# astra-vision/rain-rendering

Measured on AMD Instinct MI355X. Metric: rainy frames/sec @ 1242x375, 100 mm/hr, higher is better.
Workload: dtype f64 alpha/mask, f32 colour

## Files before the change

rain-rendering_amd/csrc/rainhip.hip:

```cpp
#include <hip/hip_runtime.h>

#include <dlfcn.h>

#include <cstddef>
#include <cstdio>
#include <cstdlib>
#include <algorithm>
#include <cstring>
#include <string>
#include <type_traits>
#include <mutex>
#include <unordered_map>
#include <vector>

#include "rainhip.h"
#include "rr_device.h"
#include "rr_prepass.h"
#include "rr_deflate.h"
#include "rr_pngrows.h"
#include "rr_particles.h"
#include "rr_lens.h"
#include "rr_resize.h"
#include "rr_convert.h"

// ... 696 lines not shown
  }
#pragma unroll
  for (int c = 0; c < NCH; c++) {
    const int y = c * 64 + lane;
    if (y < Hp) {
      uint32_t* out = sc.spans + ((int64_t)f * Hp + y) * Dp;
#pragma unroll
      for (int k = 0; k < FOV_GROUPS; k++)
        if (have[k]) out[dk[k]] = packed[k][c];
    }
  }
  if (!from_list) break;
  wave_lds_sync();
  }
}

#ifndef RR_DDA_WAVES
#define RR_DDA_WAVES 1
#endif
constexpr int DDA_WAVES = RR_DDA_WAVES;
template <int CTRL, int ROW_MASK>
__device__ inline int dpp_keep_i32(int v) { return __builtin_amdgcn_update_dpp(v, v, CTRL, ROW_MASK, 0xf, false); }
__device__ inline int wave_min_scan_i32(int v) {
  v = imin(v, dpp_keep_i32<0x111, 0xf>(v));
  v = imin(v, dpp_keep_i32<0x112, 0xf>(v));
  v = imin(v, dpp_keep_i32<0x114, 0xf>(v));
  v = imin(v, dpp_keep_i32<0x118, 0xf>(v));
  v = imin(v, dpp_keep_i32<0x142, 0xa>(v));
  v = imin(v, dpp_keep_i32<0x143, 0xc>(v));
  return v;
}
__device__ inline int wave_max_scan_i32(int v) {
  v = imax(v, dpp_keep_i32<0x111, 0xf>(v));
  v = imax(v, dpp_keep_i32<0x112, 0xf>(v));
  v = imax(v, dpp_keep_i32<0x114, 0xf>(v));
  v = imax(v, dpp_keep_i32<0x118, 0xf>(v));
  v = imax(v, dpp_keep_i32<0x142, 0xa>(v));
  v = imax(v, dpp_keep_i32<0x143, 0xc>(v));
  return v;
}

constexpr uint32_t FOV_KEY_LAST = 0xffffu;
__global__ __launch_bounds__(64 * DDA_WAVES) void k_fov_vertices(const FrameDesc* frames, Dims dm, rr_camera cam, int max_drops, int ordered, Scratch sc) {
  const int f = blockIdx.y, wave = threadIdx.x >> 6, lane = threadIdx.x & 63;
  const FrameDesc& fr = frames[f];
  const int N = cam.n_fov;
  const int i = (blockIdx.x * DDA_WAVES + wave) * 64 + lane;
  const bool act = i < fr.n_drops;
  const int64_t gi = (int64_t)f * max_drops + (act ? i : 0);
  if (fr.strategy == 1) {
    if (act) {
      sc.npts[gi] = -1;
      sc.fov_rec[gi] = make_uint4(0u, 0u, 0u, (ordered ? FOV_KEY_LAST : 0u) << 16);
    }
    return;
  }
  uint32_t* const gpix = sc.fov_pix + (int64_t)f * N * max_drops + (act ? i : 0);
  auto pixv = [&](int kk) -> uint32_t& { return gpix[(int64_t)kk * max_drops]; };
  uint32_t top_xy = 0;
  int uns = 0;
  int count_true = 0, count_false = 0;
  int ktop = 0, ytop = 1 << 30, ybot = -(1 << 30), r_first = 0;
  bool spread = false, on_map = true;
  int turns = 0, dir = 0, dir_first = 0;
  float dist = 0.f;
  if (act) {
    FovSetup32 F;
    const rr_drop d = load_drop(fr.drops + i);
    fov_setup32(d, (float)cam.fov_cos, (float)cam.fov_sin, F, uns);
    dist = sqrtf(F.pos[0] * F.pos[0] + F.pos[1] * F.pos[1] + F.pos[2] * F.pos[2]);
    float az_prev = 0.f, er_prev = 0.f, az0 = 0.f, er0 = 0.f;
    int y_prev = 0, y0v = 0;
    for (int k = 0; k < N; k++) {
      float az, er, pxf, pyf;
      fov_vertex32(F, (float)cam.radius, (float)cam.phi_cos[k], (float)cam.phi_sin[k], dm.He, dm.We, az, er, pxf, pyf, uns);
      const int ix = (int)pxf, iy = (int)pyf;
      const uint32_t vxy = (uint32_t)(ix & 0xffff) | ((uint32_t)(iy & 0xffff) << 16);
      pixv(k) = vxy;
      on_map = on_map && ix >= 0 && ix < dm.We && iy >= 0 && iy < dm.He;
      const int r = imin(imax(iy, 0), dm.He - 1);
      if (k == 0) { az0 = az; er0 = er; r_first = r; y0v = iy; }
      else {
        const bool c = fov_wrap_cnd32(az_prev, az, er_prev, er, uns);
        count_true += c ? 1 : 0;
        count_false += c ? 0 : 1;
        spread = spread || iabs(r - r_first) >= 2;
        const int sg = iy > y_prev ? 1 : (iy < y_prev ? -1 : 0);
        if (sg != 0) {
          if (dir == 0) dir_first = sg;
          else if (sg != dir) turns++;
          dir = sg;
        }
      }
      if (iy < ytop) { ytop = iy; ktop = k; top_xy = vxy; }
      ybot = imax(ybot, iy);
      az_prev = az; er_prev = er; y_prev = iy;
    }
    {
      const bool c = fov_wrap_cnd32(az_prev, az0, er_prev, er0, uns);
      count_true += c ? 1 : 0;
      count_false += c ? 0 : 1;
      const int sg = y0v > y_prev ? 1 : (y0v < y_prev ? -1 : 0);
      if (sg != 0) {
        if (dir != 0 && sg != dir) turns++;
        dir = sg;
      }
      if (dir != 0 && dir_first != 0 && dir != dir_first) turns++;
    }
  }
  if (act) {
    const uint32_t v0 = pixv(0), va = pixv(N / 2);
    const int x0v = (int)(v0 & 0xffffu), y0v = (int)(v0 >> 16), ax = (int)(va & 0xffffu) - x0v, ay = (int)(va >> 16) - y0v;
    bool sure_nc = false;
    for (int k = 1; k < N; k++) {
      const uint32_t v = pixv(k);
      sure_nc = sure_nc || poly_surely_not_collinear_step(ax, ay, (int)(v & 0xffffu) - x0v, (int)(v >> 16) - y0v);
    }
    if (!sure_nc) uns |= 256;
  }
  const bool certain_fail = (uns & 128) && !(uns & 3);
  const bool wrap = count_true == 1 || count_false == 1;
  const bool undecided = (uns & ~128) != 0 || count_true == 0 || count_false == 0 || (!wrap && !spread);
  const bool monotone = turns <= 2;
  const bool mine = act && !certain_fail && !undecided && !wrap && monotone;
  if (act && certain_fail) sc.npts[gi] = 0;
  if (act && !certain_fail && !mine) {
    const int pos = atomicAdd(&sc.fov_list_n[f], 1);
    sc.fov_list[(int64_t)f * max_drops + pos] = i;
  }
  if (mine) sc.npts[gi] = N;
  if (act) {
    uint32_t key = 0u;
    if (ordered) {
      const int bucket = (int)fminf(fmaxf(dist * 4.0f, 0.f), 62.0f);
      key = mine ? ((uint32_t)bucket << 10) | (uint32_t)imin(imax(ytop, 0), 1023) : FOV_KEY_LAST;
    }
    sc.fov_rec[gi] = make_uint4((uint32_t)ytop, (uint32_t)ybot, top_xy, (uint32_t)ktop | (mine ? 256u : 0u) | (on_map ? 512u : 0u) | (key << 16));
  }
}

__global__ __launch_bounds__(64 * DDA_WAVES) void k_fov_dda(const FrameDesc* frames, Dims dm, rr_camera cam, int max_drops, int Hp, int Dp, int cv_rule, Scratch sc) {
  const int f = blockIdx.y, wave = threadIdx.x >> 6, lane = threadIdx.x & 63;
  const FrameDesc& fr = frames[f];
  const int N = cam.n_fov;
  if (fr.strategy == 1) return;
  const int s = (blockIdx.x * DDA_WAVES + wave) * 64 + lane;
  const bool act = s < fr.n_drops;
  const int i = act ? sc.fov_order[(int64_t)f * max_drops + s] : 0;
  const uint4 dr = act ? sc.fov_rec[(int64_t)f * max_drops + i] : make_uint4(0u, 0u, 0u, 0u);
  const bool mine = act && (dr.w & 256u);
  if (__ballot(mine) == 0ull) return;
  const int ytop = (int)dr.x, ybot = (int)dr.y, ktop = (int)(dr.w & 255u);
  const uint32_t top_xy = dr.z;
  uint4* const erec = sc.fov_erec + (int64_t)f * N * max_drops + s;
  const uint32_t* const gpix = sc.fov_pix + (int64_t)f * N * max_drops + i;
  auto pixv = [&](int kk) -> uint32_t { return gpix[(int64_t)kk * max_drops]; };
  const bool cvr = cv_rule && (dr.w & 512u);
  if (mine) {
    const uint32_t vfirst = pixv(0);
    uint32_t va = vfirst;
    for (int k = 0; k < N; k++) {
      const uint32_t vb = k + 1 == N ? vfirst : pixv(k + 1);
      const int x0 = (int)(va & 0xffffu), y0 = (int)(va >> 16), x1 = (int)(vb & 0xffffu), y1 = (int)(vb >> 16);
      const bool swp = y1 < y0;
      uint32_t r[4];
      dda_edge_record(swp ? x1 : x0, swp ? y1 : y0, swp ? x0 : x1, swp ? y0 : y1, cvr, r);
      erec[(int64_t)k * max_drops] = make_uint4(r[0], r[1], r[2], r[3]);
      va = vb;
    }
  }
  auto rec = [&](int kk, uint32_t r[4]) {
    const uint4 v = erec[(int64_t)kk * max_drops];
    r[0] = v.x; r[1] = v.y; r[2] = v.z; r[3] = v.w;
  };
  DdaCursors<decltype(rec)> cur;
  if (mine) cur.init(rec, N, ktop, top_xy);
  uint32_t* out = sc.spans + (int64_t)f * Hp * Dp + s;
  const int wtop = __builtin_amdgcn_readlane(wave_min_scan_i32(mine ? imin(imax(ytop, 0), Hp) : Hp), 63);
  const int wend = imax(__builtin_amdgcn_readlane(wave_max_scan_i32(mine ? imin(imax(ybot + 1, 0), Hp) : 0), 63), wtop);
  for (int y = 0; y < wtop; y++)
    if (mine) out[(int64_t)y * Dp] = 0u;
  for (int y = wtop; y < wend; y++) {
    int lo = 1 << 30, hi = -(1 << 30);
    if (mine && y >= ytop && y <= ybot) cur.row(rec, y, lo, hi);
    const int a = imax(lo, 0), b = imin(hi, dm.We - 1);
    if (mine) out[(int64_t)y * Dp] = (y < dm.He && a <= b) ? ((uint32_t)a | ((uint32_t)(b + 1) << 16)) : 0u;
  }
  for (int y = wend; y < Hp; y++)
    if (mine) out[(int64_t)y * Dp] = 0u;
}

template <int CTRL, int ROW_MASK>
__device__ inline double dpp_move_f64(double v) {
  int lo = __double2loint(v), hi = __double2hiint(v);
  lo = __builtin_amdgcn_update_dpp(0, lo, CTRL, ROW_MASK, 0xf, true);
  hi = __builtin_amdgcn_update_dpp(0, hi, CTRL, ROW_MASK, 0xf, true);
  return __hiloint2double(hi, lo);
}
__device__ inline double row16_incl_scan_f64(double v) {
  v += dpp_move_f64<0x111, 0xf>(v);
  v += dpp_move_f64<0x112, 0xf>(v);
  v += dpp_move_f64<0x114, 0xf>(v);
  v += dpp_move_f64<0x118, 0xf>(v);
  return v;
}
__device__ inline double wave_incl_scan_f64(double v) {
  v = row16_incl_scan_f64(v);
  v += dpp_move_f64<0x142, 0xa>(v);
  v += dpp_move_f64<0x143, 0xc>(v);
  return v;
}
template <int CTRL, int ROW_MASK>
__device__ inline double dpp_keep_f64(double v) {
  int lo = __double2loint(v), hi = __double2hiint(v);
  lo = __builtin_amdgcn_update_dpp(lo, lo, CTRL, ROW_MASK, 0xf, false);
  hi = __builtin_amdgcn_update_dpp(hi, hi, CTRL, ROW_MASK, 0xf, false);
  return __hiloint2double(hi, lo);
}
__device__ inline double wave_min_scan_f64(double v) {
  v = dmin(v, dpp_keep_f64<0x111, 0xf>(v));
  v = dmin(v, dpp_keep_f64<0x112, 0xf>(v));
  v = dmin(v, dpp_keep_f64<0x114, 0xf>(v));
  v = dmin(v, dpp_keep_f64<0x118, 0xf>(v));
  v = dmin(v, dpp_keep_f64<0x142, 0xa>(v));
  v = dmin(v, dpp_keep_f64<0x143, 0xc>(v));
  return v;
}
__device__ inline double wave_max_scan_f64(double v) {
  v = dmax(v, dpp_keep_f64<0x111, 0xf>(v));
  v = dmax(v, dpp_keep_f64<0x112, 0xf>(v));
  v = dmax(v, dpp_keep_f64<0x114, 0xf>(v));
  v = dmax(v, dpp_keep_f64<0x118, 0xf>(v));
  v = dmax(v, dpp_keep_f64<0x142, 0xa>(v));
  v = dmax(v, dpp_keep_f64<0x143, 0xc>(v));
  return v;
}
__device__ inline double readlane_f64(double v, int l) {
  int lo = __double2loint(v), hi = __double2hiint(v);
  lo = __builtin_amdgcn_readlane(lo, l);
  hi = __builtin_amdgcn_readlane(hi, l);
  return __hiloint2double(hi, lo);
}

template <int DPT, int EMAX>
__global__ __launch_bounds__(1024) void k_fov_sums(const FrameDesc* frames, Dims dm, int max_drops, int Hp, int Dp, int rpb, int nchunk, Scratch sc) {
  extern __shared__ __attribute__((aligned(16))) double s_dyn[];
  const int We = dm.We;
  double2* s_P = reinterpret_cast<double2*>(s_dyn);
  double* s_wt = reinterpret_cast<double*>(s_P + (We + 1));
  const int f = blockIdx.y, band = blockIdx.x % COL_PARTS, part = blockIdx.x / COL_PARTS;
  const int half = part & 1, chunk = part >> 1;
  const int NT = blockDim.x, t = threadIdx.x, lane = t & 63, nw = NT >> 6;
  const int wave = __builtin_amdgcn_readfirstlane(t >> 6);
  const FrameDesc& fr = frames[f];
  const int n = fr.n_drops;
  const int per = (n + nchunk - 1) / nchunk;
  const int d0 = chunk * per, d1 = imin(n, d0 + per);
  if (d0 >= n) return;
  const int y0 = band * rpb, y1 = imin(dm.He, y0 + rpb);
  const int Cw = (((We + nw - 1) / nw) + 1) & ~1;
  const int cw0 = wave * Cw;
  const uint32_t* spf = sc.spans + (int64_t)f * Hp * Dp;
  uint32_t sp[DPT];
#pragma unroll
  for (int d = 0; d < DPT; d++) {
    const int i = d0 + d * NT + t;
    sp[d] = (uint32_t)((i < d1 && sc.npts[(int64_t)f * max_drops + i] > 0) ? i : max_drops);
  }
  if (t == 0) s_P[0] = make_double2(0.0, 0.0);
  double S[DPT][2];
  uint32_t any = 0;
#pragma unroll
  for (int d = 0; d < DPT; d++) S[d][0] = S[d][1] = 0.0;
  double tot0 = 0.0, tot1 = 0.0;
  double pa[EMAX][2], pb[EMAX][2];
  const bool e32 = (fr.in_types & RR_IN_ENV_F32) != 0;
  auto load_row = [&](int y) {
    const global_ptr<const double> env = as_global(static_cast<const double*>(fr.env)) + (int64_t)y * We * 3;
    const global_ptr<const double> om = as_global(static_cast<const double*>(fr.omega)) + (int64_t)y * We;
    const global_ptr<const float> envf = as_global(static_cast<const float*>(fr.env)) + (int64_t)y * We * 3;
    const global_ptr<const float> omf = as_global(static_cast<const float*>(fr.omega)) + (int64_t)y * We;
    auto E = [&](int i) { return e32 ? (double)envf[i] : env[i]; };
    auto O = [&](int i) { return e32 ? (double)omf[i] : om[i]; };
#pragma unroll
    for (int e = 0; e < EMAX; e++) {
      const int cl = e * 128 + 2 * lane, c = cw0 + cl;
      pa[e][0] = pa[e][1] = pb[e][0] = pb[e][1] = 0.0;
      if (cl < Cw && c < We) {
        const double w = O(c);
        pa[e][0] = (half ? E(c * 3 + 2) : E(c * 3 + 0)) * w;
        pa[e][1] = half ? w : E(c * 3 + 1) * w;
        if (c + 1 < We) {
          const double w1 = O(c + 1);
          pb[e][0] = (half ? E(c * 3 + 5) : E(c * 3 + 3)) * w1;
          pb[e][1] = half ? w1 : E(c * 3 + 4) * w1;
        }
      }
    }
  };
  if (y0 < y1) load_row(y0);
  for (int yq = y0; yq < y1; yq += 4) {
    uint4 q[DPT];
#pragma unroll
    for (int d = 0; d < DPT; d++)
      q[d] = make_uint4(spf[(int64_t)yq * Dp + sp[d]], spf[(int64_t)(yq + 1) * Dp + sp[d]], spf[(int64_t)(yq + 2) * Dp + sp[d]],
                        spf[(int64_t)(yq + 3) * Dp + sp[d]]);
#pragma unroll
    for (int j = 0; j < 4; j++) {
      const int y = yq + j;
      if (y >= y1) break;
      double carry[2] = {0.0, 0.0};
      double ps[EMAX][2];
#pragma unroll
      for (int e = 0; e < EMAX; e++) {
        if (e * 128 < Cw) {
#pragma unroll
          for (int k = 0; k < 2; k++) {
            const double v = wave_incl_scan_f64(pa[e][k] + pb[e][k]) + carry[k];
            ps[e][k] = v;
            carry[k] = readlane_f64(v, 63);
          }
        }
      }
      if (lane == 0) { s_wt[wave * 2 + 0] = carry[0]; s_wt[wave * 2 + 1] = carry[1]; }
      __syncthreads();
      double basev[2];
#pragma unroll
      for (int k = 0; k < 2; k++) {
        const double wt = row16_incl_scan_f64(lane < nw ? s_wt[lane * 2 + k] : 0.0);
// ... 4085 lines not shown

#define HIPCHK(call)                                                                              \
  do {                                                                                            \
    hipError_t e_ = (call);                                                                       \
    if (e_ != hipSuccess) {                                                                       \
      ctx->err = std::string(#call) + ": " + hipGetErrorString(e_);                               \
      return RR_E_HIP;                                                                            \
    }                                                                                             \
  } while (0)
#define HIPCHK_CTX(c_, call)                                                                      \
  do {                                                                                            \
    hipError_t e_ = (call);                                                                       \
    if (e_ != hipSuccess) {                                                                       \
      (c_)->err = std::string(#call) + ": " + hipGetErrorString(e_);                              \
      return RR_E_HIP;                                                                            \
    }                                                                                             \
  } while (0)

int mem_error(rr_ctx* ctx, const char* what) {
  ctx->err = std::string(what) + ": " + hipGetErrorString((hipError_t)ctx->mem.last_error);
  return RR_E_HIP;
}

template <typename T>
int dev_alloc(rr_ctx* ctx, T*& p, size_t count) {
  return ctx->mem.alloc(p, count) ? RR_OK : mem_error(ctx, "hipMalloc");
}
template <typename T>
int pin_alloc(rr_ctx* ctx, T*& p, size_t count) {
  return ctx->mem.alloc_pinned(p, count) ? RR_OK : mem_error(ctx, "hipHostMalloc");
}

template <class B, class Sync>
int reserve_after(rr_ctx* ctx, B& b, size_t need, size_t want, Sync sync) {
  return ctx->mem.reserve(b, need, want, sync) ? RR_OK : mem_error(ctx, "reserve");
}
template <class B>
int reserve(rr_ctx* ctx, B& b, size_t need, size_t want = 0, bool sync_first = true) {
  return reserve_after(ctx, b, need, want, [sync_first] { return sync_first ? (int)hipDeviceSynchronize() : 0; });
}

hipEvent_t get_event(rr_ctx* ctx) {
  if (!ctx->ev_pool.empty()) {
    hipEvent_t e = ctx->ev_pool.back();
    ctx->ev_pool.pop_back();
    return e;
  }
  hipEvent_t e;
  hipEventCreate(&e);
  return e;
}

int ring_acquire(rr_ctx* ctx, rr_ctx::DescRing& r, size_t bytes, int& idx, void*& host) {
  idx = r.next;
  r.next = (r.next + 1) % rr_ctx::DescRing::N;
  if (!r.ev[idx]) HIPCHK(hipEventCreateWithFlags(&r.ev[idx], hipEventDisableTiming));
  if (r.used[idx]) HIPCHK(hipEventSynchronize(r.ev[idx]));
  r.used[idx] = false;
  const size_t want = bytes + bytes / 2 + 4096;
  int rc = reserve(ctx, r.host[idx], bytes, want, false);
  for (int k = 0; k < rr_ctx::DescRing::N && !rc; k++) rc = reserve(ctx, r.host[k], 1, want, false);
  host = r.host[idx].p;
  return rc;
}
int ring_commit(rr_ctx* ctx, rr_ctx::DescRing& r, int idx, hipStream_t s) {
  HIPCHK(hipEventRecord(r.ev[idx], s));
  r.used[idx] = true;
  return RR_OK;
}

struct ProfScope {
  rr_ctx* ctx;
  hipStream_t s;
  ProfEntry pe;
  bool on;
  ProfScope(rr_ctx* c, hipStream_t st, const char* name) : ctx(c), s(st), on(c->prof) {
    if (on) {
      pe.name = name;
      pe.a = get_event(c);
      pe.b = get_event(c);
      hipEventRecord(pe.a, s);
    }
  }
  ~ProfScope() {
    if (on) {
      hipEventRecord(pe.b, s);
      ctx->prof_pending.push_back(pe);
    }
  }
};

void prof_collect(rr_ctx* ctx) {
  for (auto& pe : ctx->prof_pending) {
    float ms = 0.f;
    hipEventSynchronize(pe.b);
    hipEventElapsedTime(&ms, pe.a, pe.b);
    bool found = false;
    for (auto& s : ctx->prof_stats)
      if (!strcmp(s.name, pe.name)) {
        s.launches++;
        s.total_ms += ms;
        found = true;
        break;
      }
    if (!found) {
      rr_kernel_stat s;
      memset(&s, 0, sizeof(s));
      strncpy(s.name, pe.name, sizeof(s.name) - 1);
      s.launches = 1;
      s.total_ms = ms;
      ctx->prof_stats.push_back(s);
    }
    ctx->ev_pool.push_back(pe.a);
    ctx->ev_pool.push_back(pe.b);
  }
  ctx->prof_pending.clear();
}

bool fov_fast_path(const rr_ctx* ctx, const Dims& dm) {
  return !ctx->general_fov && dm.He <= HE_MAX && dm.We <= FOV_WE_MAX && (int64_t)dm.We * dm.He < (1 << 22) && ctx->cam.n_fov * 1 <= 64 &&
         ctx->cam.n_fov >= 3;
}

int ensure_scratch(rr_ctx* ctx, int n, int max_drops, const Dims& dm, bool need_comp_out) {
  const bool grow_frames = n > ctx->cap_frames;
  const bool grow_drops = max_drops > ctx->cap_drops;
  const bool dims_change = dm.H != ctx->cap_dims.H || dm.W != ctx->cap_dims.W || dm.He != ctx->cap_dims.He || dm.We != ctx->cap_dims.We;
  const bool general = !fov_fast_path(ctx, dm);
  if (grow_frames || grow_drops || dims_change || (need_comp_out && !ctx->d_comp_out) || general != ctx->scratch_general || ctx->cam.n_fov > ctx->erec_nfov) {
    HIPCHK(hipDeviceSynchronize());
    const int F = grow_frames ? n : ctx->cap_frames;
    const int D = grow_drops ? max_drops : ctx->cap_drops;
    const size_t fd = (size_t)F * (size_t)(D > 0 ? D : 1);
    const int Hp = (dm.He + 3) & ~3;
    ctx->cap_frames = ctx->cap_drops = 0;
    ctx->cap_dims = Dims{0, 0, 0, 0};
    int rc;
    if ((rc = dev_alloc(ctx, ctx->sc.plan, fd))) return rc;
    if ((rc = dev_alloc(ctx, ctx->sc.comp, fd))) return rc;
    if ((rc = dev_alloc(ctx, ctx->sc.comp32, fd))) return rc;
    if ((rc = dev_alloc(ctx, ctx->sc.npts, fd))) return rc;
    if ((rc = dev_alloc(ctx, ctx->sc.sizes, fd))) return rc;
    if ((rc = dev_alloc(ctx, ctx->sc.list_rot, fd))) return rc;
    if ((rc = dev_alloc(ctx, ctx->sc.rows_list, fd))) return rc;
    if ((rc = dev_alloc(ctx, ctx->sc.rows_sorted, fd))) return rc;
    if ((rc = dev_alloc(ctx, ctx->sc.rows_n, (size_t)F * 3))) return rc;
    if ((rc = dev_alloc(ctx, ctx->sc.rows_hist, (size_t)RW_TEX_MAX * 3 + 16))) return rc;
    ctx->sc.rows_cost = reinterpret_cast<unsigned long long*>(ctx->sc.rows_hist + RW_TEX_MAX);
    ctx->sc.rows_next = ctx->sc.rows_hist + 3 * RW_TEX_MAX;
    ctx->sc.rot_total = ctx->sc.rows_next + 1;
    if ((rc = dev_alloc(ctx, ctx->sc.rows_bounds, (size_t)RW_SHARE_MAX + 1))) return rc;
    if ((rc = dev_alloc(ctx, ctx->sc.rows_fbase, (size_t)F * RW_TEX_MAX))) return rc;
    if ((rc = dev_alloc(ctx, ctx->sc.fov_list, fd))) return rc;
    if ((rc = dev_alloc(ctx, ctx->sc.fov_erec, general ? 1 : fd * (size_t)(ctx->cam.n_fov > 0 ? ctx->cam.n_fov : RR_MAX_FOV)))) return rc;
    if ((rc = dev_alloc(ctx, ctx->sc.fov_pix, general ? 1 : fd * (size_t)(ctx->cam.n_fov > 0 ? ctx->cam.n_fov : RR_MAX_FOV)))) return rc;
    ctx->erec_nfov = ctx->cam.n_fov;
    if ((rc = dev_alloc(ctx, ctx->sc.fov_rec, general ? 1 : fd))) return rc;
    if ((rc = dev_alloc(ctx, ctx->sc.fov_order, general ? 1 : fd))) return rc;
    if ((rc = dev_alloc(ctx, ctx->sc.fov_slot, general ? 1 : fd))) return rc;
    if ((rc = dev_alloc(ctx, ctx->sc.fov_list_n, (size_t)F))) return rc;
    if ((rc = dev_alloc(ctx, ctx->sc.list_gen, fd))) return rc;
    if ((rc = dev_alloc(ctx, ctx->sc.list_slow, fd))) return rc;
    if ((rc = dev_alloc(ctx, ctx->sc.blur_items, fd * 8))) return rc;
    if ((rc = dev_alloc(ctx, ctx->sc.list_small, fd))) return rc;
    if ((rc = dev_alloc(ctx, ctx->sc.colpart, fd * COL_PARTS * 5))) return rc;
    if ((rc = dev_alloc(ctx, ctx->sc.wtab, fd * 2 * (BR_MAX + 1)))) return rc;
    if ((rc = dev_alloc(ctx, ctx->sc.wtab_big, (size_t)F * SLOW_CAP * 2 * (MAX_R + 1)))) return rc;
    if (general) {
      if ((rc = dev_alloc(ctx, ctx->sc.poly, fd * 2 * POLY_STRIDE))) return rc;
      if ((rc = dev_alloc(ctx, ctx->sc.prefix, (size_t)F * dm.He * (size_t)(dm.We + 1) * 4))) return rc;
      if ((rc = dev_alloc(ctx, ctx->sc.spans, 1))) return rc;
    } else {
      if ((rc = dev_alloc(ctx, ctx->sc.poly, 1))) return rc;
      if ((rc = dev_alloc(ctx, ctx->sc.prefix, 1))) return rc;
      const size_t per_frame = (size_t)(((D > 0 ? D : 1) + 1 + 7) & ~7) * (size_t)Hp;
      if ((rc = dev_alloc(ctx, ctx->sc.spans, (size_t)F * per_frame))) return rc;
      HIPCHK(hipMemset(ctx->sc.spans, 0, sizeof(uint32_t) * (size_t)F * per_frame));
    }
    ctx->scratch_general = general;
    ctx->scratch_hp = Hp;
    if ((rc = dev_alloc(ctx, ctx->sc.bbox, fd))) return rc;
    if ((rc = dev_alloc(ctx, ctx->sc.blended, fd))) return rc;
    {
      const size_t nct = (size_t)((dm.W + CTILE - 1) / CTILE) * ((dm.H + CTILE - 1) / CTILE);
      if ((rc = dev_alloc(ctx, ctx->sc.clist, fd * nct))) return rc;
      if ((rc = dev_alloc(ctx, ctx->sc.ccount, (size_t)F * nct))) return rc;
    }
    if ((rc = dev_alloc(ctx, ctx->sc.counts, (size_t)F * 8))) return rc;
    if ((rc = dev_alloc(ctx, ctx->sc.canon, fd))) return rc;
    if ((rc = dev_alloc(ctx, ctx->sc.bigs_list, fd))) return rc;
    if ((rc = dev_alloc(ctx, ctx->sc.bigs_n, (size_t)F))) return rc;
    if ((rc = dev_alloc(ctx, ctx->sc.tkey, fd * 2))) return rc;
    if ((rc = dev_alloc(ctx, ctx->sc.lrec, fd))) return rc;
    if ((rc = dev_alloc(ctx, ctx->sc.list_big, fd))) return rc;
    if ((rc = dev_alloc(ctx, ctx->sc.big_off, fd + F))) return rc;
    if ((rc = dev_alloc(ctx, ctx->sc.htab, fd * 2))) return rc;
    if ((rc = dev_alloc(ctx, ctx->sc.fband, (size_t)F * COL_PARTS * 2))) return rc;
    const int ntiles = ((dm.W + TILE - 1) / TILE) * ((dm.H + TILE - 1) / TILE);
    if ((rc = dev_alloc(ctx, ctx->sc.partial, (size_t)F * ntiles * 4))) return rc;
    if ((rc = dev_alloc(ctx, ctx->sc.means, (size_t)F * 4))) return rc;
    if ((rc = dev_alloc(ctx, ctx->sc.arena_need, (size_t)F))) return rc;
    if ((rc = dev_alloc(ctx, ctx->d_frames, (size_t)F))) return rc;
    if ((rc = dev_alloc(ctx, ctx->d_comp_out, (size_t)F * dm.H * dm.W * 3))) return rc;
    if (ctx->arena_cap == 0) ctx->arena_cap = (int64_t)(D > 0 ? D : 1) * 1024 + (1 << 20);
    if ((rc = dev_alloc(ctx, ctx->sc.arena, (size_t)F * (size_t)ctx->arena_cap))) return rc;
    ctx->cap_frames = F;
    ctx->cap_drops = D;
    ctx->cap_dims = dm;
  }
  return RR_OK;
}

int grow_arena(rr_ctx* ctx) {
  HIPCHK(hipDeviceSynchronize());
  unsigned long long need = 0;
  HIPCHK(hipMemcpy(&need, ctx->sc.need_max, sizeof(need), hipMemcpyDeviceToHost));
  if ((int64_t)need > ctx->arena_cap) {
    const int64_t cap = ((int64_t)need + (int64_t)need / 4 + (1 << 16) + 15) & ~15LL;
    const int F = ctx->cap_frames;
    ctx->cap_frames = 0;
    ctx->arena_cap = cap;
    int rc = dev_alloc(ctx, ctx->sc.arena, (size_t)F * (size_t)cap);
    if (rc) return rc;
    ctx->cap_frames = F;
  }
  HIPCHK(hipMemset(ctx->sc.need_max, 0, sizeof(unsigned long long)));
  return RR_OK;
}

struct PlanarOut {
  char* rgb;
  float* mask;
  int64_t rgb_stride;
  int fmt;
};

struct LensStage {
  const rr_ctx::Slot::Lens* lens;
  uint8_t* rgb;
  int64_t rgb_stride, png_stride;
};

int enqueue(rr_ctx* ctx, int n, const rr_frame_in* in, const rr_frame_out* out, hipStream_t s, int ovf_idx = 0,
            const PlanarOut* planar = nullptr, const LensStage* lens = nullptr, const LayerDesc* layer = nullptr) {
  if (!ctx->have_cam || !ctx->have_db) {
    ctx->err = "streak DB and camera must be set before rendering";
    return RR_E_STATE;
  }
  if (n <= 0 || !in || !out) {
    ctx->err = "bad frame batch";
    return RR_E_ARG;
  }
  Dims dm{in[0].H, in[0].W, in[0].He, in[0].We};
  int max_drops = 0;
  bool need_comp = false, want_png = false, any_f64_comp = false;
  for (int f = 0; f < n; f++) {
    if (in[f].H != dm.H || in[f].W != dm.W || in[f].He != dm.He || in[f].We != dm.We) {
      ctx->err = "all frames of a batch must share H,W,He,We";
      return RR_E_ARG;
    }
    if (in[f].strategy != 0 && in[f].strategy != 1) {
      ctx->err = "rendering strategy must be 0 (default) or 1 ('white'); 'naive_db' is broken in the reference (bad_weather.py:355)";
      return RR_E_ARG;
    }
    {
      const int t = in[f].in_types;
      if ((t & ~(RR_IN_BG_F32 | RR_IN_BG_U8 | RR_IN_ENV_F32 | RR_IN_RAINY_F32 | RR_IN_RAINY_U8)) || ((t & RR_IN_BG_F32) && (t & RR_IN_BG_U8)) ||
          ((t & RR_IN_RAINY_F32) && (t & RR_IN_RAINY_U8))) {
        ctx->err = "rr_frame_in.in_types: unknown bits, or two element types for one array";
        return RR_E_ARG;
      }
    }
    if (!in[f].omega && !(ctx->d_omega && ctx->omega_He == dm.He && ctx->omega_We == dm.We)) {
      ctx->err = "omega == NULL needs rr_set_solid_angles for this map size";
      return RR_E_STATE;
    }
    if (in[f].n_drops < 0 || in[f].n_drops > 65536 || !in[f].bg || !in[f].rainy_bg || !in[f].env_xyY ||
        (in[f].n_drops > 0 && !in[f].drops) || (!out[f].rainy_rgb && !(planar && out[f].mask_f64))) {
      ctx->err = "null frame pointer or n_drops outside [0, 2^16] (generator.py:425)";
      return RR_E_ARG;
    }
    if (out[f].mask_png && (!out[f].mask_f64 || !ctx->have_lut)) {
      ctx->err = "mask_png needs mask_f64 and rr_set_colormap";
      return RR_E_ARG;
    }
    if (in[f].n_drops > max_drops) max_drops = in[f].n_drops;
    if (!out[f].rainy_bg_out) need_comp = true;
    else any_f64_comp = true;
    want_png = want_png || out[f].rainy_png || out[f].mask_png;
  }
  const bool use32 = !any_f64_comp && !ctx->composite_f64;
  const bool fov32 = ctx->fov_f32 == 1 || (ctx->fov_f32 == 2 && use32);
  if (dm.H <= 0 || dm.W <= 0 || dm.He <= 0 || dm.We <= 0) {
    ctx->err = "bad frame size";
    return RR_E_ARG;
  }
  int rc = ensure_scratch(ctx, n, max_drops, dm, need_comp);
  if (rc) return rc;
  const int D = ctx->cap_drops > 0 ? ctx->cap_drops : 1;
  int ring_idx;
  void* ring_host;
  bool any_dev_count = false;
  if ((rc = ring_acquire(ctx, ctx->ring_frames, sizeof(FrameDesc) * (size_t)n, ring_idx, ring_host))) return rc;
  FrameDesc* h_frames = static_cast<FrameDesc*>(ring_host);
  for (int f = 0; f < n; f++) {
    FrameDesc& fd = h_frames[f];
    fd.bg = in[f].bg;
// ... 3136 lines not shown
```

rain-rendering_amd/csrc/rr_device.h:

```cpp
#pragma once
#include <math.h>
#include <stdint.h>

#include "rainhip.h"

#if defined(__HIPCC__)
#include <hip/hip_runtime.h>
#define RR_HD __host__ __device__ inline
#else
#define RR_HD inline
#endif

#if defined(__clang__)
#pragma clang fp contract(off)
#endif

namespace rr {

enum { KIND_BIG = 0, KIND_ROT = 1, KIND_EXT = 2 };
enum { RS_AREA = 0, RS_AREA_FAST = 1, RS_LINEAR = 2 };

struct Dims {
  int32_t H, W, He, We;
};
// ... 897 lines not shown
  if (den > iabs(dx)) {
    l = h = xa + Q + (R >= den + 1 ? 1 : 0);
  } else {
    l = xa + Q - hh + (R >= hr ? 1 : 0);
    h = xa + Q + hh + (R + hr >= dn ? 1 : 0);
    l = imax(l, imin(xa, xb));
    h = imin(h, imax(xa, xb));
  }
  if (t < den) {
    const int s = xa + ((t * dx16 + 32768) >> 16);
    l = imin(l, s);
    h = imax(h, s);
  }
}

RR_HD int mul24i(int a, int b) {
#if defined(__HIP_DEVICE_COMPILE__)
  return __mul24(a, b);
#else
  return a * b;
#endif
}
struct DdaSide {
  int xa, xb, yb, kv;
  int mn, mx;
  int Q, R, W;
  int dn, hh, tl, th, qs, rs, d16, wk;
  uint32_t n_r0, n_r1, n_r2, n_r3;
};
RR_HD void dda_take_edge(DdaSide& S, int xa, int ya, int xb, int yb, uint32_t w0, uint32_t w1) {
  S.xa = xa;
  S.xb = xb;
  S.yb = yb;
  S.mn = imin(xa, xb);
  S.mx = imax(xa, xb);
  const int den = yb - ya, dx = xb - xa;
  S.dn = 2 * den;
  S.Q = 0;
  S.R = 0;
  S.W = 32768;
  S.d16 = (int)w0;
  S.wk = (int)((w1 >> 23) & 1u);
  S.hh = (int)(w1 & 0x7ffu);
  S.tl = (int)((w1 >> 11) & 0x7ffu);
  S.th = ((w1 >> 22) & 1u) ? S.tl : S.dn - S.tl;
  S.qs = S.d16 >> 16;
  S.rs = 2 * dx - mul24i(S.qs, S.dn);
}
RR_HD void dda_pixels(const DdaSide& S, int y, int& x0, int& x1) {
  const int base = S.xa + S.Q;
  x0 = imax(base - S.hh + (S.R >= S.tl ? 1 : 0), S.mn);
  x1 = imin(base + S.hh + (S.R >= S.th ? 1 : 0), S.mx);
  if (S.wk && y < S.yb) {
    const int sx = S.xa + (S.W >> 16);
    x0 = imin(x0, sx);
    x1 = imax(x1, sx);
  }
  if (S.dn == 0) {
    x0 = S.mn;
    x1 = S.mx;
  }
}
RR_HD void dda_edge_record(int xu, int yu, int xl, int yl, bool cv, uint32_t r[4]) {
  const int den = yl - yu, dx = xl - xu;
  r[0] = r[1] = 0u;
  if (den > 0) {
    int dx16, hh, hr;
    edge_cv_consts(dx, den, dx16, hh, hr);
    r[0] = (uint32_t)dx16;
    if (!cv) r[1] = 0u | ((uint32_t)den << 11) | (1u << 22);
    else if (den > iabs(dx)) r[1] = 0u | ((uint32_t)(den + 1) << 11) | (1u << 22) | (1u << 23);
    else r[1] = (uint32_t)hh | ((uint32_t)hr << 11) | (1u << 23);
  }
  DdaSide S;
  dda_take_edge(S, xu, yu, xl, yl, r[0], r[1]);
  int x0, x1;
  dda_pixels(S, yu, x0, x1);
  r[2] = (uint32_t)(x0 & 0xffff) | ((uint32_t)(x1 & 0xffff) << 16);
  r[3] = (uint32_t)(xl & 0xffff) | ((uint32_t)(yl & 0xffff) << 16);
  if (den <= 0) r[0] = (uint32_t)(xu & 0xffff);
}
template <class E>
struct DdaCursors {
  DdaSide s0, s1;
  int used, N;
  template <int C>
  RR_HD static int next_k(int k, int n) { return C == 0 ? (k + 1 == n ? 0 : k + 1) : (k == 0 ? n - 1 : k - 1); }
  template <int C>
  RR_HD void fetch(DdaSide& S, const E& rec) const {
    uint32_t r[4];
    rec(C == 0 ? S.kv : next_k<C>(S.kv, N), r);
    S.n_r0 = r[0]; S.n_r1 = r[1]; S.n_r2 = r[2]; S.n_r3 = r[3];
  }
  template <int C, bool STEP>
  RR_HD void advance_edge(DdaSide& S, const E& rec, int& lo, int& hi) const {
    const int xa = S.xb, ya = S.yb;
    uint32_t w0 = S.n_r0;
    const uint32_t w1 = S.n_r1, w2 = S.n_r2, w3 = S.n_r3;
    S.kv = next_k<C>(S.kv, N);
    fetch<C>(S, rec);
    int xe = (int)(w3 & 0xffffu);
    const int ye = (int)(w3 >> 16);
    if (ye == ya) {
      if (C == 1) xe = (int)w0;
      w0 = 0u;
    }
    dda_take_edge(S, xa, ya, xe, ye, w0, w1);
    if (STEP) {
      lo = imin(lo, (int)(w2 & 0xffffu));
      hi = imax(hi, (int)(w2 >> 16));
      if (S.dn > 0) {
        const int carry = S.rs >= S.dn ? 1 : 0;
        S.R = S.rs - (carry ? S.dn : 0);
        S.Q = S.qs + carry;
        S.W = 32768 + S.d16;
      }
    }
  }
  template <int C>
  RR_HD void init_side(DdaSide& S, const E& rec, int ktop, uint32_t top_xy) const {
    S.xb = (int)(top_xy & 0xffffu);
    S.yb = (int)(top_xy >> 16);
    S.kv = ktop;
    fetch<C>(S, rec);
    int lo = 0, hi = 0;
    advance_edge<C, false>(S, rec, lo, hi);
  }
  RR_HD void init(const E& rec, int n, int ktop, uint32_t top_xy) {
    N = n;
    used = 2;
    init_side<0>(s0, rec, ktop, top_xy);
    init_side<1>(s1, rec, ktop, top_xy);
  }
  RR_HD static void step(DdaSide& S) {
    const int r = S.R + S.rs;
    const int carry = r >= S.dn ? 1 : 0;
    S.R = r - (carry ? S.dn : 0);
    S.Q += S.qs + carry;
    S.W += S.d16;
  }
  template <int C>
  RR_HD void side_row(DdaSide& S, const E& rec, int y, int& lo, int& hi) {
    {
      int x0, x1;
      dda_pixels(S, y, x0, x1);
      lo = imin(lo, x0);
      hi = imax(hi, x1);
    }
    step(S);
    while (y == S.yb && used < N) {
      used++;
      advance_edge<C, true>(S, rec, lo, hi);
    }
  }
  RR_HD void row(const E& rec, int y, int& lo, int& hi) {
    lo = 1 << 30;
    hi = -(1 << 30);
    side_row<0>(s0, rec, y, lo, hi);
    side_row<1>(s1, rec, y, lo, hi);
  }
};

RR_HD int poly_row_turns(const int32_t* py, int n) {
  int turns = 0, dir = 0, dir_first = 0;
  for (int k = 1; k <= n; k++) {
    const int a = py[k - 1], b = py[k == n ? 0 : k];
    const int sg = b > a ? 1 : (b < a ? -1 : 0);
    if (sg != 0) {
      if (dir == 0) dir_first = sg;
      else if (sg != dir) turns++;
      dir = sg;
    }
  }
  if (dir != 0 && dir_first != 0 && dir != dir_first) turns++;
  return turns;
}

RR_HD bool fov_fill_rule_cv_applies(const int32_t* px, const int32_t* py, int n, int n_fov, int He, int We) {
  if (n != n_fov || n < 3) return false;
  for (int k = 0; k < n; k++)
    if (px[k] < 0 || px[k] >= We || py[k] < 0 || py[k] >= He) return false;
  return poly_row_turns(py, n) <= 2;
}

RR_HD void colour_from_sums(const double S[4], double sum_omega, double ambient, double Kbgr[3]) {
  double x = S[0] / S[3], y = S[1] / S[3];
  double avg_fov_lum = S[2] / sum_omega;
  double drop_Y = 0.94 * avg_fov_lum + 0.06 * ambient;
  double Yg = ((0.31 + 0.8124) + 0.01) / 0.17697 * drop_Y;
  double X = (Yg * x) / y;
  double Z = (Yg * (1 - x - y)) / y;
  double r = (X * 0.41847 + Yg * -0.091169) + Z * 0.0009209;
  double g = (X * -0.15866 + Yg * 0.25243) + Z * -0.0025498;
  double b = (X * -0.082835 + Yg * 0.015708) + Z * 0.1786;
  Kbgr[0] = b;
  Kbgr[1] = g;
  Kbgr[2] = r;
}

RR_HD void solve8(double A[8][8], double b[8], double x[8]) {
#pragma unroll
  for (int col = 0; col < 8; col++) {
    int piv = col;
    double best = fabs(A[col][col]);
#pragma unroll
    for (int r = col + 1; r < 8; r++)
      if (fabs(A[r][col]) > best) { best = fabs(A[r][col]); piv = r; }
#pragma unroll
    for (int r = col + 1; r < 8; r++)
      if (r == piv) {
#pragma unroll
        for (int c = 0; c < 8; c++) { double t = A[col][c]; A[col][c] = A[r][c]; A[r][c] = t; }
        double t = b[col]; b[col] = b[r]; b[r] = t;
      }
#pragma unroll
    for (int r = col + 1; r < 8; r++) {
      double f = A[r][col] / A[col][col];
#pragma unroll
      for (int c = col + 1; c < 8; c++) A[r][c] = A[r][c] - f * A[col][c];
      b[r] = b[r] - f * b[col];
    }
  }
#pragma unroll
  for (int r = 7; r >= 0; r--) {
    double s = b[r];
#pragma unroll
    for (int c = r + 1; c < 8; c++) s = s - A[r][c] * x[c];
    x[r] = s / A[r][r];
  }
}

RR_HD void invert3(const double m[9], double t[9]) {
  double d = m[0] * (m[4] * m[8] - m[5] * m[7]) - m[1] * (m[3] * m[8] - m[5] * m[6]) + m[2] * (m[3] * m[7] - m[4] * m[6]);
  if (d == 0.0 || !(fabs(d) < 1.7e308)) {
    for (int i = 0; i < 9; i++) t[i] = 0.0;
    return;
  }
  d = 1.0 / d;
  t[0] = (m[4] * m[8] - m[5] * m[7]) * d;
  t[1] = (m[2] * m[7] - m[1] * m[8]) * d;
  t[2] = (m[1] * m[5] - m[2] * m[4]) * d;
  t[3] = (m[5] * m[6] - m[3] * m[8]) * d;
  t[4] = (m[0] * m[8] - m[2] * m[6]) * d;
  t[5] = (m[2] * m[3] - m[0] * m[5]) * d;
  t[6] = (m[3] * m[7] - m[4] * m[6]) * d;
  t[7] = (m[1] * m[6] - m[0] * m[7]) * d;
  t[8] = (m[0] * m[4] - m[1] * m[3]) * d;
}

RR_HD int py_slice_index(int i, int n) {
  if (i < 0) { i += n; if (i < 0) i = 0; }
  else if (i > n) i = n;
  return i;
}

RR_HD void raw_tile_key(const rr_drop& d, const DropPlan& p, uint32_t key[8]) {
  for (int k = 0; k < 8; k++) key[k] = 0u;
  key[0] = 0xffffffffu;
  if (p.status != RR_DROP_OK || (p.kind != KIND_BIG && p.kind != KIND_ROT)) return;
  if (p.tw < 0 || p.tw > 65535 || p.th < 0 || p.th > 65535) return;
  if (p.kind == KIND_BIG) {
    const double d0 = floor(d.iw1), d1 = floor(d.iw2);
    if (!(d0 > -2.0e9 && d0 < 2.0e9 && d1 > -2.0e9 && d1 < 2.0e9)) return;
    const int minx = imax(imin(d.x0, d.x1), 0), miny = imax(imin(d.y0, d.y1), 0);
    key[2] = (uint32_t)(d.x0 - minx);
    key[3] = (uint32_t)(d.y0 - miny);
    key[4] = (uint32_t)(d.x1 - minx);
    key[5] = (uint32_t)(d.y1 - miny);
    key[6] = (uint32_t)(int32_t)d0;
    key[7] = (uint32_t)(int32_t)d1;
  } else {
    uint64_t a, b;
    const double al = d.rot_cos, be = d.rot_sin;
    __builtin_memcpy(&a, &al, 8);
    __builtin_memcpy(&b, &be, 8);
    key[2] = (uint32_t)a; key[3] = (uint32_t)(a >> 32);
    key[4] = (uint32_t)b; key[5] = (uint32_t)(b >> 32);
  }
  key[0] = (uint32_t)p.kind | ((uint32_t)(p.flip & 1) << 4) | ((uint32_t)p.tex << 8);
  key[1] = (uint32_t)p.tw | ((uint32_t)p.th << 16);
}

RR_HD void plan_big_homography(const rr_drop& d, int sw, int sh, double mi[9]) {
  const double d0 = floor(d.iw1), d1 = floor(d.iw2);
  const int minx = imax(imin(d.x0, d.x1), 0), miny = imax(imin(d.y0, d.y1), 0);
  float src[4][2] = {{0.f, 0.f}, {(float)sw, 0.f}, {(float)sw, (float)sh}, {0.f, (float)sh}};
  float dst[4][2];
  dst[0][0] = (float)(d.x0 - minx);                        dst[0][1] = (float)(d.y0 - miny);
  dst[1][0] = (float)((double)(d.x0 - minx) + d0);         dst[1][1] = (float)(d.y0 - miny);
  dst[2][0] = (float)(((double)(d.x1 - minx) + d1) + 0.001); dst[2][1] = (float)(d.y1 - miny);
  dst[3][0] = (float)((double)(d.x1 - minx) + 0.001);      dst[3][1] = (float)(d.y1 - miny);
  double A[8][8], bb[8], xx[8];
#pragma unroll
  for (int i = 0; i < 8; i++)
#pragma unroll
    for (int j = 0; j < 8; j++) A[i][j] = 0.0;
#pragma unroll
  for (int i = 0; i < 4; i++) {
    double sx = src[i][0], sy = src[i][1], ddx = dst[i][0], ddy = dst[i][1];
    A[i][0] = A[i + 4][3] = sx;
    A[i][1] = A[i + 4][4] = sy;
    A[i][2] = A[i + 4][5] = 1.0;
    A[i][6] = -sx * ddx;
    A[i][7] = -sy * ddx;
    A[i + 4][6] = -sx * ddy;
    A[i + 4][7] = -sy * ddy;
// ... 264 lines not shown
```

Before: 19730.

## Precompute merged per-vertex DDA records and walk them with prefetching cursors

Replaces the per-edge record generation plus DdaCursors walk in k_fov_dda with a new FovWalk scheme. A preprocessing pass starts at the top vertex, folds horizontal edges and each edge's last-row pixel extents into packed records laid out in walk order, and emits one extra turn record, so the record buffer grows by one slot per drop. The row loop then does a fixed, branch-light update per side and prefetches the next record into registers behind a scheduling barrier. The intent is to remove the inner while-loop over edges and the dependent record loads from each row, at the cost of more packing arithmetic up front and a more intricate record encoding.

```diff
diff --git a/rain-rendering_amd/csrc/rainhip.hip b/rain-rendering_amd/csrc/rainhip.hip
--- a/rain-rendering_amd/csrc/rainhip.hip
+++ b/rain-rendering_amd/csrc/rainhip.hip
@@ -872,29 +872,21 @@
   if (__ballot(mine) == 0ull) return;
   const int ytop = (int)dr.x, ybot = (int)dr.y, ktop = (int)(dr.w & 255u);
   const uint32_t top_xy = dr.z;
-  uint4* const erec = sc.fov_erec + (int64_t)f * N * max_drops + s;
+  uint4* const erec = sc.fov_erec + (int64_t)f * (N + 1) * max_drops + s;
   const uint32_t* const gpix = sc.fov_pix + (int64_t)f * N * max_drops + i;
   auto pixv = [&](int kk) -> uint32_t { return gpix[(int64_t)kk * max_drops]; };
   const bool cvr = cv_rule && (dr.w & 512u);
-  if (mine) {
-    const uint32_t vfirst = pixv(0);
-    uint32_t va = vfirst;
-    for (int k = 0; k < N; k++) {
-      const uint32_t vb = k + 1 == N ? vfirst : pixv(k + 1);
-      const int x0 = (int)(va & 0xffffu), y0 = (int)(va >> 16), x1 = (int)(vb & 0xffffu), y1 = (int)(vb >> 16);
-      const bool swp = y1 < y0;
-      uint32_t r[4];
-      dda_edge_record(swp ? x1 : x0, swp ? y1 : y0, swp ? x0 : x1, swp ? y0 : y1, cvr, r);
-      erec[(int64_t)k * max_drops] = make_uint4(r[0], r[1], r[2], r[3]);
-      va = vb;
-    }
-  }
-  auto rec = [&](int kk, uint32_t r[4]) {
-    const uint4 v = erec[(int64_t)kk * max_drops];
+  auto rec = [&](int pos, uint32_t r[4]) {
+    const uint4 v = erec[(int64_t)pos * max_drops];
     r[0] = v.x; r[1] = v.y; r[2] = v.z; r[3] = v.w;
   };
-  DdaCursors<decltype(rec)> cur;
-  if (mine) cur.init(rec, N, ktop, top_xy);
+  FovWalk<decltype(rec)> cur;
+  if (mine) {
+    const int n_pos = fov_walk_make_records(pixv, N, imin(ktop, N - 1), cvr, [&](int pos, const uint32_t r[4]) {
+      erec[(int64_t)pos * max_drops] = make_uint4(r[0], r[1], r[2], r[3]);
+    });
+    cur.init(rec, n_pos, ytop, cvr);
+  }
   uint32_t* out = sc.spans + (int64_t)f * Hp * Dp + s;
   const int wtop = __builtin_amdgcn_readlane(wave_min_scan_i32(mine ? imin(imax(ytop, 0), Hp) : Hp), 63);
   const int wend = imax(__builtin_amdgcn_readlane(wave_max_scan_i32(mine ? imin(imax(ybot + 1, 0), Hp) : 0), 63), wtop);
@@ -5286,7 +5278,7 @@
     if ((rc = dev_alloc(ctx, ctx->sc.rows_bounds, (size_t)RW_SHARE_MAX + 1))) return rc;
     if ((rc = dev_alloc(ctx, ctx->sc.rows_fbase, (size_t)F * RW_TEX_MAX))) return rc;
     if ((rc = dev_alloc(ctx, ctx->sc.fov_list, fd))) return rc;
-    if ((rc = dev_alloc(ctx, ctx->sc.fov_erec, general ? 1 : fd * (size_t)(ctx->cam.n_fov > 0 ? ctx->cam.n_fov : RR_MAX_FOV)))) return rc;
+    if ((rc = dev_alloc(ctx, ctx->sc.fov_erec, general ? 1 : fd * (size_t)((ctx->cam.n_fov > 0 ? ctx->cam.n_fov : RR_MAX_FOV) + 1)))) return rc;
     if ((rc = dev_alloc(ctx, ctx->sc.fov_pix, general ? 1 : fd * (size_t)(ctx->cam.n_fov > 0 ? ctx->cam.n_fov : RR_MAX_FOV)))) return rc;
     ctx->erec_nfov = ctx->cam.n_fov;
     if ((rc = dev_alloc(ctx, ctx->sc.fov_rec, general ? 1 : fd))) return rc;
diff --git a/rain-rendering_amd/csrc/rr_device.h b/rain-rendering_amd/csrc/rr_device.h
--- a/rain-rendering_amd/csrc/rr_device.h
+++ b/rain-rendering_amd/csrc/rr_device.h
@@ -1073,6 +1073,155 @@
       used++;
       advance_edge<C, true>(S, rec, lo, hi);
     }
+  }
+  RR_HD void row(const E& rec, int y, int& lo, int& hi) {
+    lo = 1 << 30;
+    hi = -(1 << 30);
+    side_row<0>(s0, rec, y, lo, hi);
+    side_row<1>(s1, rec, y, lo, hi);
+  }
+};
+
+typedef uint32_t fov_rec_words __attribute__((vector_size(16)));
+struct FovWalkSide {
+  int yb;
+  int al, ah;
+  int R, W;
+  int dn, tl, th, qs, rs, d16;
+  int pos;
+  fov_rec_words nx;
+};
+template <class V, class S>
+RR_HD int fov_walk_make_records(const V& vtx, int n, int ktop, bool cv, const S& store) {
+  const int BIG = 1 << 30;
+  int p = 0;
+  int plo = BIG, phi = -BIG;
+  uint32_t q0 = 0u, q2 = 0u, q3 = 0u;
+  int qlo = BIG, qhi = -BIG;
+  bool have = false, turned = false;
+  auto put = [&](uint32_t w0, int lo, int hi, uint32_t w2, uint32_t w3) {
+    uint32_t r[4] = {w0, (uint32_t)(lo & 0xffff) | ((uint32_t)(hi & 0xffff) << 16), w2, w3};
+    store(p, r);
+    p++;
+  };
+  int k = ktop;
+  uint32_t va = vtx(k);
+  plo = phi = (int)(va & 0xffffu);
+  for (int j = 0; j < n; j++) {
+    k = k + 1 == n ? 0 : k + 1;
+    const uint32_t vb = vtx(k);
+    const int x0 = (int)(va & 0xffffu), y0 = (int)(va >> 16), x1 = (int)(vb & 0xffffu), y1 = (int)(vb >> 16);
+    va = vb;
+    if (y1 == y0) {
+      plo = imin(plo, x1);
+      phi = imax(phi, x1);
+      continue;
+    }
+    const bool down = y1 > y0;
+    const int xu = down ? x0 : x1, yu = down ? y0 : y1, xl = down ? x1 : x0, yl = down ? y1 : y0;
+    uint32_t r[4];
+    dda_edge_record(xu, yu, xl, yl, cv, r);
+    const int flo = (int)(r[2] & 0xffffu), fhi = (int)(r[2] >> 16);
+    int llo, lhi;
+    {
+      DdaSide L;
+      dda_take_edge(L, xu, yu, xl, yl, r[0], r[1]);
+      L.Q = xl - xu;
+      dda_pixels(L, yl, llo, lhi);
+    }
+    const uint32_t w2 = (r[1] & 0x3fffffu) | ((uint32_t)(yl - yu) << 22);
+    DdaSide T;
+    dda_take_edge(T, xu, yu, xl, yl, r[0], r[1]);
+    const uint32_t w3 = (uint32_t)T.rs | (((r[1] >> 22) & 1u) << 11) | ((uint32_t)xu << 16);
+    if (down) {
+      if (have) put(q0, qlo, qhi, q2, q3);
+      qlo = imin(plo, flo);
+      qhi = imax(phi, fhi);
+      plo = llo;
+      phi = lhi;
+    } else {
+      if (!turned) {
+        if (have) put(q0, qlo, qhi, q2, q3);
+        put(0u, imin(plo, llo), imax(phi, lhi), 1u << 22, 0u);
+        turned = true;
+      } else {
+        put(q0, imin(qlo, imin(plo, llo)), imax(qhi, imax(phi, lhi)), q2, q3);
+      }
+      qlo = flo;
+      qhi = fhi;
+      plo = BIG;
+      phi = -BIG;
+    }
+    q0 = r[0]; q2 = w2; q3 = w3;
+    have = true;
+  }
+  if (have) put(q0, imin(qlo, plo), imax(qhi, phi), q2, q3);
+  if (!turned) put(0u, plo, phi, 1u << 22, 0u);
+  return p;
+}
+template <class E>
+struct FovWalk {
+  FovWalkSide s0, s1;
+  int last;
+  bool wk;
+  template <int C>
+  RR_HD void fetch(FovWalkSide& S, const E& rec, int pos) const {
+    uint32_t r[4];
+    S.pos = pos;
+    rec(pos, r);
+    S.nx = fov_rec_words{r[0], r[1], r[2], r[3]};
+  }
+  template <int C>
+  RR_HD void init_side(FovWalkSide& S, const E& rec, int ytop) const {
+    S.yb = ytop;
+    S.al = S.ah = S.R = S.W = S.dn = S.tl = S.th = S.qs = S.rs = S.d16 = 0;
+    fetch<C>(S, rec, C == 0 ? 0 : last);
+  }
+  RR_HD void init(const E& rec, int n_pos, int ytop, bool cv) {
+    last = n_pos - 1;
+    wk = cv;
+    init_side<0>(s0, rec, ytop);
+    init_side<1>(s1, rec, ytop);
+  }
+  template <int C>
+  RR_HD void side_row(FovWalkSide& S, const E& rec, int y, int& lo, int& hi) const {
+    int x0 = S.al + (S.R >= S.tl ? 1 : 0), x1 = S.ah + (S.R >= S.th ? 1 : 0);
+    if (wk) {
+      const int sx = S.W >> 16;
+      x0 = imin(x0, sx);
+      x1 = imax(x1, sx);
+    }
+    {
+      const int r = S.R + S.rs;
+      const int carry = r >= S.dn ? 1 : 0;
+      S.R = r - (carry ? S.dn : 0);
+      S.al += S.qs + carry;
+      S.ah += S.qs + carry;
+      S.W += S.d16;
+    }
+    if (y == S.yb) {
+      const uint32_t w0 = S.nx[0], w1 = S.nx[1], w2 = S.nx[2], w3 = S.nx[3];
+      x0 = (int)(w1 & 0xffffu);
+      x1 = (int)(w1 >> 16);
+      const int hh = (int)(w2 & 0x7ffu), den = (int)(w2 >> 22), xa = (int)(w3 >> 16);
+      S.d16 = (int)w0;
+      S.qs = S.d16 >> 16;
+      S.tl = (int)((w2 >> 11) & 0x7ffu);
+      S.dn = 2 * den;
+      S.th = (w3 & 0x800u) ? S.tl : S.dn - S.tl;
+      S.yb += den;
+      S.rs = (int)(w3 & 0x7ffu);
+      S.R = S.rs;
+      S.al = xa + S.qs - hh;
+      S.ah = xa + S.qs + hh;
+      S.W = (int)((w3 & 0xffff0000u) + 32768u + w0);
+#if defined(__HIP_DEVICE_COMPILE__)
+      __builtin_amdgcn_sched_barrier(0);
+#endif
+      fetch<C>(S, rec, C == 0 ? imin(S.pos + 1, last) : imax(S.pos - 1, 0));
+    }
+    lo = imin(lo, x0);
+    hi = imax(hi, x1);
   }
   RR_HD void row(const E& rec, int y, int& lo, int& hi) {
     lo = 1 << 30;
```

New measurement: 20020, median of 6. +1.5%, better.
